# SonyResearch/COALA

Hardware: AMD Instinct MI355X
Metric: encode+decode GB/s over fp32 weight updates (device-resident), 1/2/4/8 GPU (higher is better)
Workload: dtype f32; 1 GPU; C3-per-GPU: 16 x resnet50_tv fp32 updates per GPU, top-k 0.01, 8-bit codes, weights mode, encode+decode batched as 2 concurrent sub-batches; layout=resnet50_tv, clients_per_gpu=16, elements_per_client=25610152, segments_per_client=267, mode=weights, global_clients=16, bits=8, inflight_steps=1, parallelism=replicas1

## Files before the change

coala_amd/compression/_lib.py:

```python
import ctypes
import os
import threading

from .. import _build

COALAC_FLAG_FORCE_EXACT = 1
COALAC_FLAG_GENERIC_SELECT = 2
COALAC_FLAG_STAMPS = 4
COALAC_FLAG_NO_FORK = 8
COALAC_AGG_DIV = 0
COALAC_AGG_RECIP = 1
COALAC_AGG_SUM = 2
COALAC_AGGD_CODES = 0
COALAC_AGGD_PACKED = 1
COALAC_AGGD_BLOCK = 2
COALAC_AGGS_ENTRIES = 0
COALAC_AGGS_COMPACT = 1
AGGD_DEPTH = 4

ERRORS = {
    -1: "COALAC_EINVAL",
    -2: "COALAC_EBITS",
    -3: "COALAC_EWORKSPACE",
    -4: "COALAC_EHIP",
    -5: "COALAC_EDEVICE",
    -6: "COALAC_ENOMEM",
}

_P = ctypes.c_void_p
_U64 = ctypes.c_uint64
_I = ctypes.c_int
SIGNATURES = [
    ("coalac_version", _I, []),
    ("coalac_last_error", ctypes.c_char_p, []),
    ("coalac_plan_create", _I, [_P, _I, _I, ctypes.POINTER(_P)]),
    ("coalac_plan_destroy", _I, [_P]),
    ("coalac_plan_query", _I, [_P, ctypes.POINTER(_U64), ctypes.POINTER(_U64), ctypes.POINTER(_U64),
                               ctypes.POINTER(_U64)]),
    ("coalac_encode", _I, [_P, _P, _P, _P, _P, _P, _P, _P, _P, _U64, ctypes.c_uint, _P]),
    ("coalac_encode_segptr", _I, [_P, _P, _P, _P, _P, _P, _P, _P, _P, _U64, ctypes.c_uint, _P]),
    ("coalac_decode", _I, [_P, _P, _P, _P, _P, _P, _P, _P, _P]),
    ("coalac_ef_accumulate", _I, [_P, _P, _P, _P, _P, _P]),
    ("coalac_ef_commit", _I, [_P, _P, _P, _P, _P, _P, _P, _P]),
    ("coalac_plan_packed_bytes", _I, [_P, ctypes.POINTER(_U64)]),
    ("coalac_pack", _I, [_P, _P, _P, _P, _U64, _P]),
    ("coalac_unpack", _I, [_P, _P, _U64, _P, _P, _P, _P]),
    ("coalac_plan_dense_packed_bytes", _I, [_P, ctypes.POINTER(_U64)]),
    ("coalac_pack_dense", _I, [_P, _P, _P, _U64, _P]),
    ("coalac_unpack_dense", _I, [_P, _P, _U64, _P, _P]),
    ("coalac_decode_packed", _I, [_P, _P, _U64, _P, _P, _P, _P, _P]),
    ("coalac_encode_block", _I, [_P, _P, _P, _P, _P, _P, _P, _U64, _P]),
    ("coalac_decode_block", _I, [_P, _P, _U64, _P, _P, _P, _P, _P]),
    ("coalac_encode_sr", _I, [_P, _P, _P, _P, _P, _P, _P, _P, _U64, _U64, ctypes.c_uint, _P]),
    ("coalac_encode_block_sr", _I, [_P, _P, _P, _P, _P, _P, _P, _U64, _U64, _P]),
    ("coalac_encode_ev", _I, [_P, _P, _P, _P, _P, _P, _P, _P, _P, _U64, ctypes.c_uint, _P, _P]),
    ("coalac_decode_ev", _I, [_P, _P, _P, _P, _P, _P, _P, _P, _P, _P]),
    ("coalac_aggregate", _I, [_P, _I, _P, _P, _P, _P, _P, _P, ctypes.c_float, _I, _P, _P, _P, _P]),
    ("coalac_aggregate_ev", _I, [_P, _I, _P, _P, _P, _P, _P, _P, ctypes.c_float, _I, _P, _P, _P, _P, _P]),
    ("coalac_aggregate_dense", _I, [_P, _I, _I, _P, _U64, _P, _P, _P, ctypes.c_float, _I, _P, _P, _P, _P]),
    ("coalac_aggregate_uploads", _I, [_P, _I, _I, _P, _P, _U64, _P, _P, _P, _P, _P, ctypes.c_float, _I, _P, _P, _P, _P]),
    ("coalac_gather", _I, [_P, _I, _I, _P, _P]),
    ("coalac_workspace_fallbacks", _I, [_P, _P, _P, ctypes.POINTER(_I)]),
    ("coalac_debug_stamps", _I, [_P, _P, _P, ctypes.POINTER(ctypes.c_uint64), _I]),
    ("coalac_debug_brackets", _I, [_P, _P, _P, ctypes.POINTER(ctypes.c_uint32), ctypes.POINTER(ctypes.c_uint32), _I]),
]

ABI_VERSION = 11
ADDED_IN_ABI_11 = ("coalac_encode_sr", "coalac_encode_block_sr")


class CodecError(RuntimeError):
    pass


class SegDesc(ctypes.Structure):
    _fields_ = [("in_off", _U64), ("n", _U64), ("k", _U64), ("out_off", _U64)]


_lock = threading.Lock()
_lib = None


def lib_path():
    return os.environ.get("COALAC_LIB") or _build.LIB


def load(build_if_missing=True):
    global _lib
    if _lib is not None:
        return _lib
    with _lock:
        if _lib is not None:
            return _lib
        path = lib_path()
        if not os.environ.get("COALAC_LIB") and (
                not os.path.exists(path) or (build_if_missing and _build.stale() and _can_build())):
            if not build_if_missing:
                raise CodecError(f"HIP codec library not found at {path}; run __graft_entry__.build()")
            _build.build()
        lib = ctypes.CDLL(path)
        lib.coalac_version.restype, lib.coalac_version.argtypes = _I, []
        v = lib.coalac_version()
        if v != ABI_VERSION:
            raise CodecError(f"libcoalac ABI version {v} != expected {ABI_VERSION} ({path}: rebuild it from this tree)")
        for name, res, args in SIGNATURES:
            if name in ADDED_IN_ABI_11 and not hasattr(lib, name):
                continue
            fn = getattr(lib, name)
            fn.restype = res
            fn.argtypes = args
        _lib = lib
        return lib


def _can_build():
    try:
        _build.hipcc()
        return True
    except RuntimeError:
        return False

# ... 6 lines not shown
```

coala_amd/compression/plan.py:

```python
import contextlib
import ctypes
from dataclasses import dataclass

import torch

from . import _lib
from .spec import RAW_BITS, UNIT, VALID_BITS, SegmentTable, SubTable


@dataclass
class Encoded:
    idx: torch.Tensor
    vals: torch.Tensor
    mn: torch.Tensor
    scale: torch.Tensor
    ustart: torch.Tensor = None
    packed: torch.Tensor = None

    FIELDS = ("idx", "vals", "mn", "scale", "ustart")

    def to(self, device, non_blocking=False):
        return Encoded(*(None if t is None else t.to(device, non_blocking=non_blocking)
                         for t in (self.idx, self.vals, self.mn, self.scale, self.ustart, self.packed)))

# ... 19 lines not shown

def _stream_handle(stream):
    s = torch.cuda.current_stream() if stream is None else stream
    return ctypes.c_void_p(s.cuda_stream)


class CodecPlan:

    def __init__(self, sizes, ratio, bits=8, clients=1, device=None, table=None):
        if bits not in VALID_BITS:
            raise ValueError(f"bits must be one of {VALID_BITS}, got {bits}")
        self.table = SegmentTable(sizes, ratio, clients) if table is None else table
        self.bits = int(bits)
        self.device = torch.device("cuda", torch.cuda.current_device() if device is None
                                   else torch.device(device).index or 0)
        self._lib = _lib.load()
        segs = self.table.segs
        arr = (_lib.SegDesc * len(segs))()
        for i, (a, b, c, d) in enumerate(segs.tolist()):
            arr[i] = _lib.SegDesc(a, b, c, d)
        h = ctypes.c_void_p()
        with torch.cuda.device(self.device):
            _lib.check(self._lib.coalac_plan_create(arr, len(segs), self.bits, ctypes.byref(h)),
                       "coalac_plan_create")
        self._h = h
        ws, tk, span, nu = (ctypes.c_uint64() for _ in range(4))
        _lib.check(self._lib.coalac_plan_query(h, ctypes.byref(ws), ctypes.byref(tk), ctypes.byref(span),
                                               ctypes.byref(nu)), "coalac_plan_query")
        self.ws_bytes = ws.value
        self.total_k, self.span, self.n_units = tk.value, span.value, nu.value
        if self.total_k != self.table.total_k:
            raise _lib.CodecError(f"plan total_k {self.total_k} != table {self.table.total_k}")
        if self.n_units != self.table.n_units:
            raise _lib.CodecError(f"plan n_units {self.n_units} != table {self.table.n_units}")
        segs = self.table.segs
        self.dense = bool(len(segs)) and bool((segs[:, 1] == segs[:, 2]).all())
        self.implied_idx = self.dense and getattr(self.table, "ratio", None) is not None and self.table.ratio >= 1.0

    @classmethod
    def from_segments(cls, segs, bits=8, device=None):
        return cls(None, None, bits, device=device, table=SubTable(segs))

    def close(self):
        h, self._h = getattr(self, "_h", None), None
        if h is not None and h.value:
            with torch.cuda.device(self.device):
                self._lib.coalac_plan_destroy(h)

    def __del__(self):
        try:
            self.close()
        except Exception:
            pass

    @property
    def n_segments(self):
        return self.table.n_segments

    @property
    def vals_dtype(self):
        return torch.float32 if self.bits == RAW_BITS else torch.uint8

    def empty_flat(self):
        return torch.empty(self.span, dtype=torch.float32, device=self.device)

    def empty_encoded(self, with_idx=None):
        if with_idx is None:
            with_idx = not self.implied_idx
        if not with_idx:
            vb = 4 if self.bits == RAW_BITS else 1
            T = self.n_segments
            buf = torch.empty((vb * self.total_k + 15) // 16 * 16 + 8 * T, dtype=torch.uint8, device=self.device)
            o = (vb * self.total_k + 15) // 16 * 16
            return Encoded(torch.empty(0, dtype=torch.int32, device=self.device), buf[:vb * self.total_k].view(self.vals_dtype),
                           buf[o:o + 4 * T].view(torch.float32), buf[o + 4 * T:o + 8 * T].view(torch.float32), None)
        geo = self.__dict__.get("_enc_geometry")
        if geo is None:
            K, T, U = self.total_k, self.n_segments, self.n_units
            vb = 4 if self.bits == RAW_BITS else 1
            views, o = [], 0
            dts = (torch.int32, self.vals_dtype, torch.float32, torch.float32, torch.int32)
            for nbytes, dt in zip((4 * K, vb * K, 4 * T, 4 * T, 4 * U), dts):
                views.append((o, nbytes, dt))
                o = (o + nbytes + 15) // 16 * 16
            geo = self._enc_geometry = (max(o, 16), tuple(views))
        buf = torch.empty(geo[0], dtype=torch.uint8, device=self.device)
        return Encoded(*[buf[a:a + n].view(dt) for a, n, dt in geo[1]])

    def empty_workspace(self):
        return torch.empty(self.ws_bytes, dtype=torch.uint8, device=self.device)

    def _check_flat(self, t, name, need=None):
        if t is None:
            return
        need = self.span if need is None else need
        if t.device != self.device or t.dtype != torch.float32 or not t.is_contiguous():
            raise ValueError(f"{name}: need a contiguous float32 tensor on {self.device}, got "
                             f"{t.dtype} on {t.device} (contiguous={t.is_contiguous()})")
        if t.numel() < need:
            raise ValueError(f"{name}: {t.numel()} elements < required {need}")
        if t.data_ptr() % 16:
            raise ValueError(f"{name}: storage must be 16-byte aligned")

    def _check_encoded(self, e):
        want = ((e.idx, torch.int32, 0 if self.dense and e.idx.numel() == 0 else self.total_k),
                (e.vals, self.vals_dtype, self.total_k),
# ... 567 lines not shown
```

coala_amd/csrc/coalac.hip:

```cpp
#pragma clang fp contract(off)

#include <hip/hip_runtime.h>

#include <algorithm>
#include <cmath>
#include <cstdarg>
#include <cstdio>
#include <cstdlib>
#include <cstring>
#include <mutex>
#include <string>
#include <type_traits>
#include <vector>

#include "../../include/coalac.h"

namespace {

constexpr int BLOCK = 256;
constexpr int WAVES = BLOCK / 64;
constexpr uint32_t UNIT = 4096;
constexpr uint32_t UNIT_SHIFT = 12;
constexpr uint32_t UNIT_IT = UNIT / 256;
constexpr uint32_t SMALL_MAX = 4096;
// ... 1806 lines not shown
    const uint32_t so = gx + qp;
    if (valid) {
      pst(P, P.eqpre + lb + i, ex);
      pst(P, P.outoff + lb + i, so);
      if (P.ustart_out != nullptr) pst(P, P.ustart_out + sd.unit_begin + i, so);
      const uint32_t rawu = raw_path | (zero_tie && quota > 0 ? 1u : 0u);
      P.uemit[lb + i] = make_uint4(T, rt | (rawu << 31), __float_as_uint(mn), __float_as_uint(scale));
    }
  }
}

template <int NT, bool DELTA, bool RAW>
DEV void segment_select(const Params& P, uint32_t li, SelSmem& S) {
  const uint32_t t = threadIdx.x;
  const uint32_t s = P.large_list[li];
  const SegDev sd = P.lsegs[li];
  const uint4 st = P.sstate[li];
  const uint32_t lb = sd.lu_begin, nu = sd.unit_end - sd.unit_begin;
  STAMP(P, li, 0);
  uint32_t T = 0, rt = 0, fp_rank = NONE, fn_rank = NONE;
  float gmn = qnan(), gmx = qnan();
  const bool zero_tie = st.w == 2;
  bool done;
  if (zero_tie) {
    const uint32_t g0 = sd.g_begin, ng = (nu + GU - 1) / GU;
    const uint32_t tk = P.tlo[lb] & KEY_MAX;
    gmn = t < ng ? P.gmm[2 * (g0 + t)] : qnan();
    gmx = t < ng ? P.gmm[2 * (g0 + t) + 1] : qnan();
    for (uint32_t i = t; i < nu; i += NT) S.ge[i] = P.gtC[lb + i] | (P.cntZ[lb + i] << 16);
    __syncthreads();
    T = tk;
    rt = st.z;
    fp_rank = rt > 0 ? 0u : NONE;
    if (tk != 0u) zero_tie_ranks<NT>(P, lb, nu, S, fp_rank, fn_rank);
    done = true;
  } else {
    done = st.w == 0 && select_from_groups<NT>(P, sd, lb, nu, st, S, T, rt, fp_rank, fn_rank, gmn, gmx);
  }
  uint32_t raw_path = 0;
  STAMP(P, li, 1);
  if (!done) select_fallback<NT, DELTA>(P, s, sd, S, T, rt, fp_rank, fn_rank, gmn, gmx, raw_path);
  STAMP(P, li, 10);
  select_finish<NT, RAW>(P, s, sd, S, done, zero_tie, raw_path, T, rt, fp_rank, fn_rank, gmn, gmx);
  STAMP(P, li, 12);
}

template <bool DELTA, bool RAW, int NT = SEL_NT>
__global__ __launch_bounds__(NT) void k_select(Params P) {
  __shared__ SelSmem S;
  segment_select<NT, DELTA, RAW>(P, blockIdx.x, S);
}

constexpr uint32_t EMIT_UPW = 4u;
constexpr uint32_t EMIT_UPW_LAT = 1u;

template <bool DELTA, bool RAW>
DEV void emit_raw_unit(const Params& P, const UnitDev& L, uint32_t T, uint32_t rt, uint32_t eqp, uint64_t obase,
                       float mn, float scale) {
  const uint32_t lane = lane_id();
  uint32_t eqc = 0, outc = 0;
  raw_unit_rows<DELTA>(P, L, [&](uint32_t row, float4 v) {
    const float xs[4] = {v.x, v.y, v.z, v.w};
    const uint32_t e0 = (row * 64 + lane) * 4;
    bool gt[4], tie[4], sel[4];
    uint32_t tpre = 0, spre = 0, ntie = 0, nsel = 0;
    uint64_t tb[4];
#pragma unroll
    for (int j = 0; j < 4; ++j) {
      const uint32_t key = fkey(xs[j]);
      const bool ok = e0 + j < L.len;
      gt[j] = ok && key > T;
      tie[j] = ok && key == T;
      tb[j] = __ballot(tie[j]);
      tpre += mbcnt(tb[j]);
      ntie += (uint32_t)__popcll(tb[j]);
    }
    uint32_t mine = 0;
#pragma unroll
    for (int j = 0; j < 4; ++j) {
      sel[j] = gt[j] || (tie[j] && eqp + eqc + tpre + mine < rt);
      mine += tie[j] ? 1u : 0u;
    }
    uint64_t sb[4];
#pragma unroll
    for (int j = 0; j < 4; ++j) {
      sb[j] = __ballot(sel[j]);
      spre += mbcnt(sb[j]);
      nsel += (uint32_t)__popcll(sb[j]);
    }
    uint32_t k = 0;
#pragma unroll
    for (int j = 0; j < 4; ++j) {
      if (sel[j]) {
        const uint64_t o = obase + outc + spre + k;
        P.idx[o] = (int32_t)(L.start + e0 + j);
        store_val<RAW>(P, o, xs[j], mn, scale);
        ++k;
      }
    }
    eqc += ntie;
    outc += nsel;
  });
}

template <bool DELTA, bool RAW, uint32_t UPW, uint32_t TR>
DEV void emit_units(const Params& P, uint32_t lu0, uint32_t lu1, uint32_t stride) {
  const uint32_t lane = lane_id();
  auto unit = [&](uint32_t g) { return lu0 + g * stride; };
  const uint32_t ng = lu0 < lu1 ? min(UPW, (lu1 - lu0 + stride - 1) / stride) : 0u;
  const uint32_t lug = unit(min(lane, ng - 1));
  uint32_t nCg, startg, eqpg, oog, Tg, rtg, stg;
  uint64_t sog;
  float mng, scg;
  uint2 rec0[UPW];
  if constexpr (UPW == 1) {
    const uint32_t nCr = P.cntC[lug];
    startg = P.lunits[lug].start;
    sog = P.lunits[lug].out_off;
    eqpg = P.eqpre[lug];
    oog = P.outoff[lug];
    const uint4 ue = P.uemit[lug];
    const uint64_t r0 = (uint64_t)lu0 * P.ccap;
    rec0[0] = make_uint2(P.cpos[r0 + lane], P.cval[r0 + lane]);
    nCg = min(nCr, P.ccap);
    Tg = ue.x;
    rtg = ue.y & 0x7FFFFFFFu;
    stg = ue.y >> 31;
    mng = RAW ? 0.0f : __uint_as_float(ue.z);
    scg = RAW ? 0.0f : __uint_as_float(ue.w);
  } else {
    nCg = min(P.cntC[lug], P.ccap);
    startg = P.lunits[lug].start;
    sog = P.lunits[lug].out_off;
    eqpg = P.eqpre[lug];
    oog = P.outoff[lug];
    const uint4 ue = P.uemit[lug];
    Tg = ue.x;
    rtg = ue.y & 0x7FFFFFFFu;
    stg = ue.y >> 31;
    mng = RAW ? 0.0f : __uint_as_float(ue.z);
    scg = RAW ? 0.0f : __uint_as_float(ue.w);
#pragma unroll
    for (uint32_t g = 0; g < UPW; ++g) {
      const uint32_t lu = unit(min(g, ng - 1)), nC = rl(nCg, g);
      const uint32_t last = nC ? nC - 1 : 0u;
      const uint64_t r0 = (uint64_t)lu * P.ccap;
      rec0[g] = make_uint2(P.cpos[r0 + min(lane, last)], P.cval[r0 + min(lane, last)]);
    }
  }
#pragma unroll
  for (uint32_t g = 0; g < UPW; ++g) {
    const uint32_t nC = rl(nCg, g);
    if (g < ng && rl(stg, g) != 0) {
      const uint64_t so = ((uint64_t)rl((uint32_t)(sog >> 32), g) << 32) | rl((uint32_t)sog, g);
      emit_raw_unit<DELTA, RAW>(P, P.lunits[unit(g)], rl(Tg, g), rl(rtg, g), rl(eqpg, g), so + rl(oog, g),
                                __uint_as_float(rl(__float_as_uint(mng), g)), __uint_as_float(rl(__float_as_uint(scg), g)));
    } else if (g < ng && nC != 0) {
      const uint32_t lu = unit(g);
      const uint32_t T = rl(Tg, g), rt = rl(rtg, g), eqp = rl(eqpg, g);
      const float mn = __uint_as_float(rl(__float_as_uint(mng), g));
      const float scale = __uint_as_float(rl(__float_as_uint(scg), g));
      const uint64_t so = ((uint64_t)rl((uint32_t)(sog >> 32), g) << 32) | rl((uint32_t)sog, g);
      const uint64_t obase = so + rl(oog, g);
      const uint32_t start = rl(startg, g);
      const uint64_t r0 = (uint64_t)lu * P.ccap;
      uint32_t eqc = 0, outc = 0;
      auto row = [&](uint32_t i0, uint2 rec) {
        const uint32_t i = i0 + lane;
        const bool valid = i < nC;
        const float x = __uint_as_float(rec.y);
        const uint32_t key = fkey(x);
        const bool e = valid && key == T;
        const uint64_t eb = __ballot(e);
        const uint32_t rank = eqp + eqc + mbcnt(eb);
        eqc += (uint32_t)__popcll(eb);
        const bool sel = valid && (key > T || (e && rank < rt));
        const uint64_t sb = __ballot(sel);
        if (sel) {
          const uint64_t o = obase + outc + mbcnt(sb);
          P.idx[o] = (int32_t)(start + rec.x);
          store_val<RAW>(P, o, x, mn, scale);
        }
        outc += (uint32_t)__popcll(sb);
      };
      row(0, rec0[g]);
      for (uint32_t i0 = 64; i0 < nC; i0 += 64 * TR) {
        uint2 rb[TR];
#pragma unroll
        for (uint32_t b = 0; b < TR; ++b) {
          const uint32_t ic = min(i0 + b * 64 + lane, nC - 1);
          if (i0 + b * 64 < nC) rb[b] = make_uint2(P.cpos[r0 + ic], P.cval[r0 + ic]);
        }
#pragma unroll
        for (uint32_t b = 0; b < TR; ++b)
          if (i0 + b * 64 < nC) row(i0 + b * 64, rb[b]);
      }
    }
  }
}

template <bool DELTA, bool RAW, uint32_t UPW, uint32_t TR>
__global__ __launch_bounds__(BLOCK) void k_emit(Params P) {
  const uint32_t wv = threadIdx.x >> 6;
  const uint32_t t0 = blockIdx.x * WAVES * UPW;
  if (t0 + wv >= P.n_lunits) return;
  const bool st = blockIdx.x < P.nseg;
  if (st) STAMP(P, blockIdx.x, 13);
  emit_units<DELTA, RAW, UPW, TR>(P, t0 + wv, min(t0 + WAVES * UPW, P.n_lunits), WAVES);
  if (st) STAMP(P, blockIdx.x, 14);
}

constexpr int DECODE_LDS_WPE = 5;
constexpr int DECODE_LDS_WPE_BASE = 4;
constexpr uint32_t DECODE_QROWS = 8u;
constexpr uint32_t DECODE_QROWS_BASE = 4u;
constexpr int DECODE_NT = 256;
constexpr uint32_t DECODE_WPU_LAT = 2u;
constexpr int DECODE_SAUX_LAT = 0;

template <bool RAW, bool HASBASE, uint32_t WPU, uint32_t QROWS, int SAUX, bool XCD, uint32_t NCH = 1>
__global__ __launch_bounds__(DECODE_NT, HASBASE ? DECODE_LDS_WPE_BASE : DECODE_LDS_WPE) void k_decode_lds(Params P) {
  constexpr uint32_t DW = DECODE_NT / 64, RPW = UNIT_IT / WPU, NPASS = RPW / QROWS;
  constexpr uint32_t QSH = QROWS == 2u ? 9u : QROWS == 4u ? 10u : QROWS == 8u ? 11u : 12u, QM = (1u << QSH) - 1u;
  static_assert((QROWS << 8) == (1u << QSH) && RPW % QROWS == 0 && NPASS >= 1, "tile pass geometry");
  __shared__ float4 qtile[DW][QROWS * 64];
  const uint32_t lane = lane_id(), wv = threadIdx.x >> 6;
  const uint32_t wid = (XCD ? xcd_block(blockIdx.x) : blockIdx.x) * DW + wv;
  const uint32_t u = wid / WPU, pass0 = (wid % WPU) * NPASS;
  if (u >= P.n_units) return;
  float4* tile = qtile[wv];
  float* tf = reinterpret_cast<float*>(tile);
#pragma unroll
  for (uint32_t it = 0; it < QROWS; ++it) tile[it * 64 + lane] = make_float4(0.0f, 0.0f, 0.0f, 0.0f);
  const UnitDev U = P.units[u];
  uint32_t lo = P.ustart[u];
  uint32_t hi = P.ustart[min(u + 1, P.n_units - 1)];
  const float mn = RAW ? 0.0f : P.cmn[U.seg], sc = RAW ? 0.0f : P.cscale[U.seg];
  lo = min(lo, U.k);
  hi = max(lo, min(min(U.last ? U.k : hi, U.k), lo + U.len));
// ... 1336 lines not shown
  std::vector<uint4> groups, gseg;
};

size_t place_tables(const PlanTables& T, Params& P, uint8_t* host, const uint8_t* dev) {
  Carver c{host};
  auto put = [&](auto*& dst, const auto& v) {
    using E = typename std::decay_t<decltype(v)>::value_type;
    static_assert(std::is_same<decltype(dst), const E*&>::value, "table and pointer types differ");
    E* h = c.take<E>(v.size());
    if (!host) return;
    if (!v.empty()) memcpy(h, v.data(), sizeof(E) * v.size());
    dst = reinterpret_cast<const E*>(dev + (reinterpret_cast<uint8_t*>(h) - host));
  };
  put(P.segs, T.segs);
  put(P.units, T.units);
  put(P.lunits, T.lunits);
  put(P.small_list, T.small_list);
  put(P.large_list, T.large_list);
  put(P.lsegs, T.lsegs);
  put(P.ssegs, T.ssegs);
  put(P.groups, T.groups);
  put(P.gseg, T.gseg);
  return c.off + 256;
}

template <typename F>
auto with_flags(F&& f) {
  return f();
}
template <typename F, typename... Rest>
auto with_flags(F&& f, bool flag, Rest... rest) {
  if (flag) return with_flags([&](auto... t) { return f(std::true_type{}, t...); }, rest...);
  return with_flags([&](auto... t) { return f(std::false_type{}, t...); }, rest...);
}
template <typename F>
auto with_agg_mode(int mode, F&& f) {
  if (mode == COALAC_AGG_RECIP) return f(std::integral_constant<int, COALAC_AGG_RECIP>{});
  if (mode == COALAC_AGG_SUM) return f(std::integral_constant<int, COALAC_AGG_SUM>{});
  return f(std::integral_constant<int, COALAC_AGG_DIV>{});
}

constexpr uint32_t FORK_MIN_LUNITS = 16384;

}

struct coalac_plan {
  int device = -1;
  int bits = 8;
  bool dense = false;
  bool dense_empty = false;
  bool encode_latency = false;
  bool decode_latency = false;
  bool high_ratio = false;
  bool small_1k = false;
  bool fork_sized = false;
  uint64_t span = 0, total_k = 0, ws_bytes = 0;
  uint64_t dense_words = 0;
  const uint64_t* dense_pw = nullptr;
  Params proto{};
  void* meta = nullptr;
  std::vector<SegDev> hsegs;
  hipStream_t side = nullptr;
  hipEvent_t fork = nullptr, join = nullptr;
  std::mutex mu;
};

namespace {

int check_device(coalac_plan_t plan) {
  int dev = -1;
  HIP_CHECK(hipGetDevice(&dev));
  if (dev != plan->device)
    return fail(COALAC_EDEVICE, "current device %d differs from the plan's device %d", dev, plan->device);
  return COALAC_OK;
}

uintptr_t addr_bits(const void* a, const void* b = nullptr, const void* c = nullptr) {
  return reinterpret_cast<uintptr_t>(a) | reinterpret_cast<uintptr_t>(b) | reinterpret_cast<uintptr_t>(c);
}

void set_payload(Params& P, const int32_t* d_idx, const void* d_vals, const float* d_mn, const float* d_scale) {
  P.cidx = d_idx;
  P.cvals = d_vals;
  P.cmn = d_mn;
  P.cscale = d_scale;
}

int launched() {
  HIP_CHECK(hipGetLastError());
  return COALAC_OK;
}

struct Marks {
  void* const* ev;
  int n;
  int at(int i, hipStream_t st) const {
    if (ev != nullptr && i < n && ev[i] != nullptr) HIP_CHECK(hipEventRecord(static_cast<hipEvent_t>(ev[i]), st));
    return COALAC_OK;
  }
};

#define MARK(i)                         \
  do {                                  \
    const int rc_ = marks.at((i), st);  \
    if (rc_) return rc_;                \
  } while (0)
// ... 44 lines not shown
    lk.lock();
    if (plan->side == nullptr) {
      if (hipStreamCreateWithFlags(&plan->side, hipStreamNonBlocking) != hipSuccess ||
          hipEventCreateWithFlags(&plan->fork, hipEventDisableTiming) != hipSuccess ||
          hipEventCreateWithFlags(&plan->join, hipEventDisableTiming) != hipSuccess)
        return fail(COALAC_EHIP, "creating the plan's side stream / events failed: %s",
                    hipGetErrorString(hipGetLastError()));
    }
  }
  MARK(0);
  if (fork) {
    HIP_CHECK(hipEventRecord(plan->fork, st));
    HIP_CHECK(hipStreamWaitEvent(plan->side, plan->fork, 0));
    hipLaunchKernelGGL((k_small<DELTA, RAW>), dim3(P.n_small), dim3(BLOCK), 0, plan->side, P);
    HIP_CHECK(hipEventRecord(plan->join, plan->side));
  }
  if (presel && !small_in_scan)
    hipLaunchKernelGGL((k_presel<DELTA, RAW>), dim3(P.n_large + P.n_small), dim3(BLOCK), 0, st, P);
  else if (P.n_large && lat)
    hipLaunchKernelGGL((k_sample<DELTA, RAW, SAMPLE_NT_LAT>), dim3(P.n_large), dim3(SAMPLE_NT_LAT), 0, st, P);
  else if (P.n_large)
    hipLaunchKernelGGL((k_sample<DELTA, RAW, BLOCK>), dim3(P.n_large), dim3(BLOCK), 0, st, P);
  MARK(1);
  if (small_in_scan) {
    Q.scan_small = P.n_small;
    const dim3 gs(ceil_div(P.n_lunits, SCAN_NT_LAT / 64) + P.n_small);
    if (plan->small_1k)
      hipLaunchKernelGGL((k_scan<DELTA, RAW, true, SCAN_WPE_LAT_1K, SCAN_NB_LAT, SCAN_NT_LAT, SMALL_MAX_LATENCY>), gs,
                         dim3(SCAN_NT_LAT), 0, st, Q);
    else
      hipLaunchKernelGGL((k_scan<DELTA, RAW, true, SCAN_WPE_LAT, SCAN_NB_LAT, SCAN_NT_LAT>), gs, dim3(SCAN_NT_LAT), 0, st,
                         Q);
  } else if (P.n_lunits) {
    hipLaunchKernelGGL((k_scan<DELTA, RAW, false, SCAN_WPE, SCAN_NB, SCAN_NT>), dim3(ceil_div(P.n_lunits, SCAN_NT / 64)),
                       dim3(SCAN_NT), 0, st, Q);
  }
  MARK(2);
  if (P.n_large && lat) {
    hipLaunchKernelGGL((k_ghist<GHIST_NT_LAT, true>), dim3(P.n_groups), dim3(GHIST_NT_LAT), 0, st, P);
    hipLaunchKernelGGL((k_gwin<GWIN_NT_LAT, true>), dim3(P.n_groups), dim3(GWIN_NT_LAT), 0, st, P);
    hipLaunchKernelGGL((k_select<DELTA, RAW, SEL_NT_LAT>), dim3(P.n_large), dim3(SEL_NT_LAT), 0, st, P);
  } else if (P.n_large) {
    with_flags(
        [&](auto hr) {
          hipLaunchKernelGGL((k_ghist<BLOCK, false, hr.value>), dim3(P.n_groups), dim3(BLOCK), 0, st, P);
          hipLaunchKernelGGL((k_gwin<BLOCK, false, hr.value>), dim3(P.n_groups), dim3(BLOCK), 0, st, P);
        },
        plan->high_ratio);
    hipLaunchKernelGGL((k_select<DELTA, RAW>), dim3(P.n_large), dim3(SEL_NT), 0, st, P);
  }
  MARK(3);
  if (P.n_large)
    with_flags(
        [&](auto l, auto hr) {
          constexpr uint32_t UPW = l.value ? EMIT_UPW_LAT : EMIT_UPW, TR = hr.value ? 4u : 1u;
          hipLaunchKernelGGL((k_emit<DELTA, RAW, UPW, TR>), dim3(ceil_div(P.n_lunits, UPW * WAVES)), dim3(BLOCK), 0, st, P);
        },
        lat, plan->high_ratio);
  if (fork) HIP_CHECK(hipStreamWaitEvent(st, plan->join, 0));
  MARK(4);
  return COALAC_OK;
}

int encode_impl(coalac_plan_t plan, const float* d_in, const float* const* d_inptr, const float* d_base,
                int32_t* d_idx, void* d_vals, float* d_mn, float* d_scale, uint32_t* d_ustart, void* d_ws,
                uint64_t ws_bytes, unsigned flags, void* stream, const Marks& marks) {
  if (!plan) return fail(COALAC_EINVAL, "coalac_encode: plan is NULL");
  if (plan->proto.nseg == 0) return COALAC_OK;
  if (!d_mn || !d_scale) return fail(COALAC_EINVAL, "coalac_encode: mn/scale pointers are NULL");
  if (plan->span && !d_in && !d_inptr) return fail(COALAC_EINVAL, "coalac_encode: input pointer is NULL");
  if (plan->total_k && (!(d_idx || plan->dense) || !d_vals))
    return fail(COALAC_EINVAL, "coalac_encode: idx/vals pointers are NULL (idx may be NULL for a dense plan only)");
  if (addr_bits(d_in, d_base) & 15) return fail(COALAC_EINVAL, "coalac_encode: input/base must be 16-byte aligned");
  if (addr_bits(d_ustart) & 3) return fail(COALAC_EINVAL, "coalac_encode: ustart must be 4-byte aligned");
  if (!d_ws || ws_bytes < plan->ws_bytes)
    return fail(COALAC_EWORKSPACE, "coalac_encode: workspace %llu < required %llu", (unsigned long long)ws_bytes,
                (unsigned long long)plan->ws_bytes);
  int rc = check_device(plan);
  if (rc) return rc;
  Params P = plan->proto;
  P.in = d_in;
  P.inptr = d_inptr;
  P.base = d_base;
  P.idx = d_idx;
  P.vals = d_vals;
  P.mn = d_mn;
  P.scale = d_scale;
  P.ustart_out = d_ustart;
  P.flags = flags;
  carve_workspace(P, plan->dense, d_ws);
  if (!(flags & COALAC_FLAG_STAMPS)) P.stamps = nullptr;
  hipStream_t st = static_cast<hipStream_t>(stream);
  rc = with_flags(
      [&](auto delta, auto raw) {
        return plan->dense ? launch_dense_encode<delta.value, raw.value>(P, plan, st, marks)
                           : launch_encode<delta.value, raw.value>(P, plan, st, marks);
      },
      d_base != nullptr, plan->bits == 32);
  return rc ? rc : launched();
}

template <bool RAW, bool HB, bool HR>
void launch_decode_lds(const Params& P, coalac_plan_t plan, hipStream_t st) {
  constexpr uint32_t DW = DECODE_NT / 64, NCH = HR ? 8u : 1u;
  if (plan->decode_latency) {
    constexpr uint32_t W = DECODE_WPU_LAT, Q = HB ? DECODE_QROWS_BASE : UNIT_IT / DECODE_WPU_LAT;
    hipLaunchKernelGGL((k_decode_lds<RAW, HB, W, (Q < 8u ? Q : 8u), DECODE_SAUX_LAT, false, NCH>),
                       dim3(ceil_div(P.n_units * W, DW)), dim3(DECODE_NT), 0, st, P);
  } else {
    hipLaunchKernelGGL((k_decode_lds<RAW, HB, 1u, HB ? DECODE_QROWS_BASE : DECODE_QROWS, STORE_AUX, true, NCH>),
                       dim3(ceil_div(P.n_units, DW)), dim3(DECODE_NT), 0, st, P);
// ... 116 lines not shown
      for (uint32_t g0 = 0; g0 < nu; g0 += GU) {
        T.groups.push_back(make_uint4((uint32_t)T.large_list.size(), d.lu_begin + g0, std::min(GU, nu - g0), (uint32_t)s));
        T.gseg.push_back(make_uint4(d.lu_begin, nu, (uint32_t)g.k, d.g_begin));
      }
    }
    (large ? T.large_list : T.small_list).push_back((uint32_t)s);
    (large ? T.lsegs : T.ssegs).push_back(d);
    T.segs[s] = d;
    if (g.n) {
      span = std::max<uint64_t>(span, g.in_off + g.n);
      total_k = std::max<uint64_t>(total_k, g.out_off + g.k);
      in_r.push_back({g.in_off, g.in_off + g.n});
      out_r.push_back({g.out_off, g.out_off + g.k});
    }
  }
  if (T.lunits.size() >= (1ull << 32) / UNIT)
    return fail(COALAC_EINVAL, "plan too large (%zu large units)", T.lunits.size());
  auto overlaps = [](std::vector<std::pair<uint64_t, uint64_t>>& r) {
    std::sort(r.begin(), r.end());
    for (size_t i = 1; i < r.size(); ++i)
      if (r[i].first < r[i - 1].second) return true;
    return false;
  };
  if (overlaps(in_r)) return fail(COALAC_EINVAL, "segment input ranges overlap");
  if (overlaps(out_r)) return fail(COALAC_EINVAL, "segment output ranges overlap");

  int dev = 0;
  HIP_CHECK(hipGetDevice(&dev));
  coalac_plan* p = new coalac_plan();
  p->device = dev;
  p->bits = bits;
  p->span = span;
  p->total_k = total_k;
  p->hsegs = T.segs;
  Params& M = p->proto;
  M.nseg = (uint32_t)nseg;
  M.n_small = (uint32_t)T.small_list.size();
  M.n_large = (uint32_t)T.large_list.size();
  M.n_units = (uint32_t)T.units.size();
  M.n_lunits = (uint32_t)T.lunits.size();
  M.n_groups = (uint32_t)T.groups.size();
  M.levels = bits == 32 ? 0.0f : (float)((1u << bits) - 1u);
  double rmax = 0.0;
  for (const SegDev& d : T.lsegs) rmax = std::max(rmax, (double)d.k / (double)d.n);
  uint32_t ccap = (uint32_t)align_up((size_t)(UNIT * std::min(1.0, 2.0 * rmax + 0.05) + 256.0), 64);
  if (const char* e = getenv("COALAC_CCAP")) ccap = (uint32_t)atoi(e);
  M.ccap = std::max<uint32_t>(STAGE_CAP, std::min<uint32_t>(UNIT, ccap));
  p->dense = true;
  for (const SegDev& d : T.segs) p->dense = p->dense && d.k == d.n;
  for (const SegDev& d : T.segs) p->dense_empty = p->dense_empty || d.unit_begin == d.unit_end;
  p->encode_latency = M.n_lunits <= LATENCY_PLAN_UNITS;
  p->decode_latency = decode_latency;
  p->high_ratio = rmax > HIGH_RATIO;
  p->small_1k = small_max <= SMALL_MAX_LATENCY;
  p->fork_sized = M.n_small && M.n_lunits >= FORK_MIN_LUNITS;
  p->ws_bytes = carve_workspace(M, p->dense, nullptr);
  std::vector<uint64_t> dense_pw;
  if (p->dense && bits != 32) {
    dense_pw.reserve(T.segs.size());
    for (const SegDev& d : T.segs) {
      dense_pw.push_back(p->dense_words);
      p->dense_words += ((uint64_t)d.n * (uint64_t)bits + 31u) / 32u;
    }
  }

  const size_t tables = place_tables(T, M, nullptr, nullptr);
  const size_t bytes = tables + align_up(sizeof(uint64_t) * dense_pw.size(), 256);
  std::vector<uint8_t> host(bytes, 0);
  hipError_t e = hipMalloc(&p->meta, bytes);
  if (e != hipSuccess) {
    delete p;
    return fail(COALAC_ENOMEM, "hipMalloc(%zu) for plan metadata failed: %s", bytes, hipGetErrorString(e));
  }
  place_tables(T, M, host.data(), static_cast<const uint8_t*>(p->meta));
  if (!dense_pw.empty()) {
    memcpy(host.data() + tables, dense_pw.data(), sizeof(uint64_t) * dense_pw.size());
    p->dense_pw = reinterpret_cast<const uint64_t*>(static_cast<const uint8_t*>(p->meta) + tables);
  }
  e = hipMemcpy(p->meta, host.data(), bytes, hipMemcpyHostToDevice);
  if (e != hipSuccess) {
    (void)hipFree(p->meta);
    delete p;
    return fail(COALAC_EHIP, "hipMemcpy of plan metadata failed: %s", hipGetErrorString(e));
  }
  *out = p;
  return COALAC_OK;
}

int coalac_plan_destroy(coalac_plan_t plan) {
  if (!plan) return COALAC_OK;
  int cur = 0;
  if (hipGetDevice(&cur) == hipSuccess && cur != plan->device) (void)hipSetDevice(plan->device);
  hipError_t e = hipFree(plan->meta);
  if (plan->side) (void)hipStreamDestroy(plan->side);
  if (plan->fork) (void)hipEventDestroy(plan->fork);
  if (plan->join) (void)hipEventDestroy(plan->join);
  if (cur != plan->device) (void)hipSetDevice(cur);
  delete plan;
  if (e != hipSuccess) return fail(COALAC_EHIP, "hipFree failed: %s", hipGetErrorString(e));
  return COALAC_OK;
}

int coalac_plan_query(coalac_plan_t plan, uint64_t* ws_bytes, uint64_t* total_k, uint64_t* span, uint64_t* n_units) {
  if (!plan) return fail(COALAC_EINVAL, "coalac_plan_query: plan is NULL");
  if (ws_bytes) *ws_bytes = plan->ws_bytes;
  if (total_k) *total_k = plan->total_k;
  if (span) *span = plan->span;
  if (n_units) *n_units = plan->proto.n_units;
  return COALAC_OK;
}

int coalac_encode_ev(coalac_plan_t plan, const float* d_in, const float* d_base, int32_t* d_idx,
                     void* d_vals, float* d_mn, float* d_scale, uint32_t* d_ustart, void* d_ws, uint64_t ws_bytes,
                     unsigned flags, void* stream, void* const* events) {
  return encode_impl(plan, d_in, nullptr, d_base, d_idx, d_vals, d_mn, d_scale, d_ustart, d_ws, ws_bytes, flags, stream,
                     Marks{events, 5});
}

int coalac_encode_segptr(coalac_plan_t plan, const float* const* d_seg_in, const float* d_base, int32_t* d_idx,
                         void* d_vals, float* d_mn, float* d_scale, uint32_t* d_ustart, void* d_ws, uint64_t ws_bytes,
                         unsigned flags, void* stream) {
  if (plan && plan->proto.nseg && !d_seg_in) return fail(COALAC_EINVAL, "coalac_encode_segptr: d_seg_in is NULL");
  return encode_impl(plan, nullptr, d_seg_in, d_base, d_idx, d_vals, d_mn, d_scale, d_ustart, d_ws, ws_bytes, flags,
                     stream, Marks{nullptr, 0});
}

int coalac_encode(coalac_plan_t plan, const float* d_in, const float* d_base, int32_t* d_idx, void* d_vals,
                  float* d_mn, float* d_scale, uint32_t* d_ustart, void* d_ws, uint64_t ws_bytes, unsigned flags,
                  void* stream) {
  return coalac_encode_ev(plan, d_in, d_base, d_idx, d_vals, d_mn, d_scale, d_ustart, d_ws, ws_bytes, flags, stream,
                          nullptr);
}

int coalac_decode_ev(coalac_plan_t plan, const int32_t* d_idx, const void* d_vals, const float* d_mn,
                     const float* d_scale, const uint32_t* d_ustart, const float* d_base, float* d_out, void* stream,
                     void* const* events) {
  if (!plan) return fail(COALAC_EINVAL, "coalac_decode: plan is NULL");
  if (plan->proto.n_units == 0) return COALAC_OK;
  if (!d_out) return fail(COALAC_EINVAL, "coalac_decode: output pointer is NULL");
  if (plan->total_k && (!(plan->dense || (d_idx && d_ustart)) || !d_vals))
    return fail(COALAC_EINVAL, "coalac_decode: idx/vals/ustart pointers are NULL (a sparse plan needs the per-unit "
                "starts of wire v2)");
  if (plan->total_k && plan->bits != 32 && (!d_mn || !d_scale))
    return fail(COALAC_EINVAL, "coalac_decode: mn/scale pointers are NULL");
  if (addr_bits(d_out, d_base) & 15) return fail(COALAC_EINVAL, "coalac_decode: output/base must be 16-byte aligned");
  if (addr_bits(d_ustart) & 3) return fail(COALAC_EINVAL, "coalac_decode: ustart must be 4-byte aligned");
  int rc = check_device(plan);
  if (rc) return rc;
  Params P = plan->proto;
  set_payload(P, d_idx, d_vals, d_mn, d_scale);
  P.base = d_base;
  P.out = d_out;
  P.ustart = d_ustart;
  hipStream_t st = static_cast<hipStream_t>(stream);
  const bool raw = plan->bits == 32, hb = d_base != nullptr;
  const Marks marks{events, 3};
  MARK(0);
  MARK(1);
  if (plan->dense)
    with_flags(
        [&](auto r, auto h, auto x) {
// ... 522 lines not shown
```

include/coalac.h:

```cpp
#ifndef COALAC_H
#define COALAC_H

#include <stdint.h>

#ifdef __cplusplus
extern "C" {
#endif

#define COALAC_ABI_VERSION 11

enum {
  COALAC_OK = 0,
  COALAC_EINVAL = -1,
  COALAC_EBITS = -2,
  COALAC_EWORKSPACE = -3,
  COALAC_EHIP = -4,
  COALAC_EDEVICE = -5,
  COALAC_ENOMEM = -6
};

enum {
  COALAC_FLAG_FORCE_EXACT = 1,
  COALAC_FLAG_GENERIC_SELECT = 2,
  COALAC_FLAG_STAMPS = 4,
  COALAC_FLAG_NO_FORK = 8
};

typedef struct coalac_seg {
  uint64_t in_off;
  uint64_t n;
  uint64_t k;
  uint64_t out_off;
} coalac_seg_t;

typedef struct coalac_plan* coalac_plan_t;

int coalac_version(void);
const char* coalac_last_error(void);

int coalac_plan_create(const coalac_seg_t* h_segs, int nseg, int bits, coalac_plan_t* out);
int coalac_plan_destroy(coalac_plan_t plan);

int coalac_plan_query(coalac_plan_t plan, uint64_t* ws_bytes, uint64_t* total_k, uint64_t* span, uint64_t* n_units);

int coalac_encode(coalac_plan_t plan, const float* d_in, const float* d_base, int32_t* d_idx,
                  void* d_vals, float* d_mn, float* d_scale, uint32_t* d_ustart, void* d_ws, uint64_t ws_bytes,
                  unsigned flags, void* stream);

int coalac_encode_segptr(coalac_plan_t plan, const float* const* d_seg_in, const float* d_base, int32_t* d_idx,
                         void* d_vals, float* d_mn, float* d_scale, uint32_t* d_ustart, void* d_ws, uint64_t ws_bytes,
                         unsigned flags, void* stream);

int coalac_decode(coalac_plan_t plan, const int32_t* d_idx, const void* d_vals, const float* d_mn,
                  const float* d_scale, const uint32_t* d_ustart, const float* d_base, float* d_out, void* stream);

int coalac_ef_accumulate(coalac_plan_t plan, const float* d_in, const float* const* d_seg_in, const float* d_base,
                         float* d_resid, void* stream);
int coalac_ef_commit(coalac_plan_t plan, const int32_t* d_idx, const void* d_vals, const float* d_mn,
                     const float* d_scale, const uint32_t* d_ustart, float* d_resid, void* stream);

int coalac_plan_packed_bytes(coalac_plan_t plan, uint64_t* bytes);
int coalac_pack(coalac_plan_t plan, const int32_t* d_idx, const void* d_vals, void* d_packed, uint64_t packed_bytes,
                void* stream);
int coalac_unpack(coalac_plan_t plan, const void* d_packed, uint64_t packed_bytes, const uint32_t* d_ustart,
                  int32_t* d_idx, void* d_vals, void* stream);

int coalac_plan_dense_packed_bytes(coalac_plan_t plan, uint64_t* bytes);
int coalac_pack_dense(coalac_plan_t plan, const void* d_vals, void* d_packed, uint64_t packed_bytes, void* stream);
int coalac_unpack_dense(coalac_plan_t plan, const void* d_packed, uint64_t packed_bytes, void* d_vals, void* stream);
int coalac_decode_packed(coalac_plan_t plan, const void* d_packed, uint64_t packed_bytes, const float* d_mn,
                         const float* d_scale, const float* d_base, float* d_out, void* stream);

int coalac_encode_block(coalac_plan_t plan, const float* d_in, const float* const* d_seg_in, const float* d_base,
                        float* d_bmn, float* d_bscale, void* d_packed, uint64_t packed_bytes, void* stream);
int coalac_decode_block(coalac_plan_t plan, const void* d_packed, uint64_t packed_bytes, const float* d_bmn,
                        const float* d_bscale, const float* d_base, float* d_out, void* stream);

int coalac_encode_sr(coalac_plan_t plan, const float* d_in, const float* const* d_seg_in, const float* d_base,
                     void* d_vals, float* d_mn, float* d_scale, void* d_ws, uint64_t ws_bytes, uint64_t seed,
                     unsigned flags, void* stream);
int coalac_encode_block_sr(coalac_plan_t plan, const float* d_in, const float* const* d_seg_in, const float* d_base,
                           float* d_bmn, float* d_bscale, void* d_packed, uint64_t packed_bytes, uint64_t seed,
                           void* stream);

int coalac_encode_ev(coalac_plan_t plan, const float* d_in, const float* d_base, int32_t* d_idx,
                     void* d_vals, float* d_mn, float* d_scale, uint32_t* d_ustart, void* d_ws, uint64_t ws_bytes,
                     unsigned flags, void* stream, void* const* events);
int coalac_decode_ev(coalac_plan_t plan, const int32_t* d_idx, const void* d_vals, const float* d_mn,
                     const float* d_scale, const uint32_t* d_ustart, const float* d_base, float* d_out, void* stream,
                     void* const* events);

enum { COALAC_AGG_DIV = 0, COALAC_AGG_RECIP = 1, COALAC_AGG_SUM = 2 };
int coalac_aggregate(coalac_plan_t plan, int clients, const int32_t* d_idx, const void* d_vals,
                     const float* d_mn, const float* d_scale, const uint32_t* d_ustart, const float* d_weights,
                     float total, int mode, const uint8_t* d_avg_mask, const float* d_base, float* d_out,
                     void* stream);
// ... 32 lines not shown
```

Before: 2790 GB/s.

## Make emit units-per-wave selectable and prefetch candidate rows speculatively

The emit kernel's units-per-wave becomes a per-plan setting (default 2, overridable via env var or API) instead of the fixed 4, which raises the number of blocks launched. For multi-unit waves, the first two 64-wide candidate rows of every unit are now loaded up front without bounds clamping, and the high-ratio extra rows are prefetched before the emit loop. This is meant to hide global-load latency behind earlier issue. It costs more registers per thread, which may reduce occupancy.

```diff
diff --git a/coala_amd/compression/_lib.py b/coala_amd/compression/_lib.py
--- a/coala_amd/compression/_lib.py
+++ b/coala_amd/compression/_lib.py
@@ -37,6 +37,8 @@
     ("coalac_plan_destroy", _I, [_P]),
     ("coalac_plan_query", _I, [_P, ctypes.POINTER(_U64), ctypes.POINTER(_U64), ctypes.POINTER(_U64),
                                ctypes.POINTER(_U64)]),
+    ("coalac_plan_emit_upw", _I, [_P, ctypes.POINTER(_I), ctypes.POINTER(_I)]),
+    ("coalac_plan_set_emit_upw", _I, [_P, _I]),
     ("coalac_encode", _I, [_P, _P, _P, _P, _P, _P, _P, _P, _P, _U64, ctypes.c_uint, _P]),
     ("coalac_encode_segptr", _I, [_P, _P, _P, _P, _P, _P, _P, _P, _P, _U64, ctypes.c_uint, _P]),
     ("coalac_decode", _I, [_P, _P, _P, _P, _P, _P, _P, _P, _P]),
@@ -66,7 +68,7 @@
 ]
 
 ABI_VERSION = 11
-ADDED_IN_ABI_11 = ("coalac_encode_sr", "coalac_encode_block_sr")
+ADDED_IN_ABI_11 = ("coalac_encode_sr", "coalac_encode_block_sr", "coalac_plan_emit_upw", "coalac_plan_set_emit_upw")
 
 
 class CodecError(RuntimeError):
diff --git a/coala_amd/compression/plan.py b/coala_amd/compression/plan.py
--- a/coala_amd/compression/plan.py
+++ b/coala_amd/compression/plan.py
@@ -95,6 +95,30 @@
             self.close()
         except Exception:
             pass
+
+    EMIT_UPW_CHOICES = (2, 4, 8)
+
+    def _emit_query(self):
+        fn = getattr(self._lib, "coalac_plan_emit_upw", None)
+        if fn is None:
+            raise _lib.CodecError("the loaded codec library has no coalac_plan_emit_upw (built before the plan field)")
+        upw, batch = ctypes.c_int(), ctypes.c_int()
+        _lib.check(fn(self._h, ctypes.byref(upw), ctypes.byref(batch)), "coalac_plan_emit_upw")
+        return upw.value, bool(batch.value)
+
+    @property
+    def emit_upw(self):
+        return self._emit_query()[0]
+
+    @emit_upw.setter
+    def emit_upw(self, upw):
+        if int(upw) not in self.EMIT_UPW_CHOICES:
+            raise ValueError(f"emit_upw must be one of {self.EMIT_UPW_CHOICES}, got {upw}")
+        _lib.check(self._lib.coalac_plan_set_emit_upw(self._h, int(upw)), "coalac_plan_set_emit_upw")
+
+    @property
+    def encode_batch(self):
+        return self._emit_query()[1]
 
     @property
     def n_segments(self):
diff --git a/coala_amd/csrc/coalac.hip b/coala_amd/csrc/coalac.hip
--- a/coala_amd/csrc/coalac.hip
+++ b/coala_amd/csrc/coalac.hip
@@ -1882,6 +1882,13 @@
 }
 
 constexpr uint32_t EMIT_UPW = 4u;
+inline uint32_t emit_upw_for(bool high_ratio, double kept_per_unit, uint32_t ccap) {
+  (void)high_ratio;
+  (void)kept_per_unit;
+  (void)ccap;
+  return 2u;
+}
+constexpr uint32_t EMIT_SPEC_ROWS = 2u;
 constexpr uint32_t EMIT_UPW_LAT = 1u;
 
 template <bool DELTA, bool RAW>
@@ -1942,7 +1949,9 @@
   uint32_t nCg, startg, eqpg, oog, Tg, rtg, stg;
   uint64_t sog;
   float mng, scg;
-  uint2 rec0[UPW];
+  constexpr uint32_t SR = UPW == 1 ? 1u : EMIT_SPEC_ROWS;
+  uint2 rec0[UPW][SR];
+  uint2 rec1[UPW][TR];
   if constexpr (UPW == 1) {
     const uint32_t nCr = P.cntC[lug];
     startg = P.lunits[lug].start;
@@ -1951,7 +1960,7 @@
     oog = P.outoff[lug];
     const uint4 ue = P.uemit[lug];
     const uint64_t r0 = (uint64_t)lu0 * P.ccap;
-    rec0[0] = make_uint2(P.cpos[r0 + lane], P.cval[r0 + lane]);
+    rec0[0][0] = make_uint2(P.cpos[r0 + lane], P.cval[r0 + lane]);
     nCg = min(nCr, P.ccap);
     Tg = ue.x;
     rtg = ue.y & 0x7FFFFFFFu;
@@ -1959,23 +1968,38 @@
     mng = RAW ? 0.0f : __uint_as_float(ue.z);
     scg = RAW ? 0.0f : __uint_as_float(ue.w);
   } else {
-    nCg = min(P.cntC[lug], P.ccap);
+    uint32_t nCr = P.cntC[lug];
     startg = P.lunits[lug].start;
     sog = P.lunits[lug].out_off;
     eqpg = P.eqpre[lug];
     oog = P.outoff[lug];
     const uint4 ue = P.uemit[lug];
+#pragma unroll
+    for (uint32_t g = 0; g < UPW; ++g) {
+      const uint64_t r0 = (uint64_t)unit(min(g, ng - 1)) * P.ccap;
+#pragma unroll
+      for (uint32_t b = 0; b < SR; ++b)
+        rec0[g][b] = make_uint2(P.cpos[r0 + b * 64 + lane], P.cval[r0 + b * 64 + lane]);
+    }
+    uint32_t uy = ue.y;
+    asm volatile("" : "+v"(nCr), "+v"(uy)::"memory");
+    nCg = min(nCr, P.ccap);
     Tg = ue.x;
-    rtg = ue.y & 0x7FFFFFFFu;
-    stg = ue.y >> 31;
+    rtg = uy & 0x7FFFFFFFu;
+    stg = uy >> 31;
     mng = RAW ? 0.0f : __uint_as_float(ue.z);
     scg = RAW ? 0.0f : __uint_as_float(ue.w);
 #pragma unroll
     for (uint32_t g = 0; g < UPW; ++g) {
-      const uint32_t lu = unit(min(g, ng - 1)), nC = rl(nCg, g);
-      const uint32_t last = nC ? nC - 1 : 0u;
-      const uint64_t r0 = (uint64_t)lu * P.ccap;
-      rec0[g] = make_uint2(P.cpos[r0 + min(lane, last)], P.cval[r0 + min(lane, last)]);
+      const uint32_t nC = rl(nCg, g);
+      if (g < ng && rl(stg, g) == 0 && nC > 64 * SR) {
+        const uint64_t r0 = (uint64_t)unit(g) * P.ccap;
+#pragma unroll
+        for (uint32_t b = 0; b < TR; ++b) {
+          const uint32_t ic = min(64 * (SR + b) + lane, nC - 1);
+          rec1[g][b] = make_uint2(P.cpos[r0 + ic], P.cval[r0 + ic]);
+        }
+      }
     }
   }
 #pragma unroll
@@ -2013,8 +2037,17 @@
         }
         outc += (uint32_t)__popcll(sb);
       };
-      row(0, rec0[g]);
-      for (uint32_t i0 = 64; i0 < nC; i0 += 64 * TR) {
+#pragma unroll
+      for (uint32_t b = 0; b < SR; ++b)
+        if (b * 64 < nC) row(b * 64, rec0[g][b]);
+      if constexpr (UPW != 1) {
+        if (nC > 64 * SR) {
+#pragma unroll
+          for (uint32_t b = 0; b < TR; ++b)
+            if (64 * (SR + b) < nC) row(64 * (SR + b), rec1[g][b]);
+        }
+      }
+      for (uint32_t i0 = 64 * (UPW == 1 ? 1u : SR + TR); i0 < nC; i0 += 64 * TR) {
         uint2 rb[TR];
 #pragma unroll
         for (uint32_t b = 0; b < TR; ++b) {
@@ -3457,6 +3490,7 @@
   bool encode_latency = false;
   bool decode_latency = false;
   bool high_ratio = false;
+  uint32_t emit_upw = EMIT_UPW;
   bool small_1k = false;
   bool fork_sized = false;
   uint64_t span = 0, total_k = 0, ws_bytes = 0;
@@ -3607,11 +3641,12 @@
   MARK(3);
   if (P.n_large)
     with_flags(
-        [&](auto l, auto hr) {
-          constexpr uint32_t UPW = l.value ? EMIT_UPW_LAT : EMIT_UPW, TR = hr.value ? 4u : 1u;
+        [&](auto l, auto hr, auto wide, auto widest) {
+          constexpr uint32_t UPW = l.value ? EMIT_UPW_LAT : !wide.value ? 2u : widest.value ? 8u : 4u;
+          constexpr uint32_t TR = hr.value ? 4u : 1u;
           hipLaunchKernelGGL((k_emit<DELTA, RAW, UPW, TR>), dim3(ceil_div(P.n_lunits, UPW * WAVES)), dim3(BLOCK), 0, st, P);
         },
-        lat, plan->high_ratio);
+        lat, plan->high_ratio, plan->emit_upw >= 4u, plan->emit_upw == 8u);
   if (fork) HIP_CHECK(hipStreamWaitEvent(st, plan->join, 0));
   MARK(4);
   return COALAC_OK;
@@ -3834,6 +3869,13 @@
   p->encode_latency = M.n_lunits <= LATENCY_PLAN_UNITS;
   p->decode_latency = decode_latency;
   p->high_ratio = rmax > HIGH_RATIO;
+  uint64_t kept_large = 0;
+  for (const SegDev& d : T.lsegs) kept_large += d.k;
+  p->emit_upw = emit_upw_for(p->high_ratio, M.n_lunits ? (double)kept_large / (double)M.n_lunits : 0.0, M.ccap);
+  if (const char* e = getenv("COALAC_EMIT_UPW")) {
+    const int v = atoi(e);
+    if (v == 2 || v == 4 || v == 8) p->emit_upw = (uint32_t)v;
+  }
   p->small_1k = small_max <= SMALL_MAX_LATENCY;
   p->fork_sized = M.n_small && M.n_lunits >= FORK_MIN_LUNITS;
   p->ws_bytes = carve_workspace(M, p->dense, nullptr);
@@ -3889,6 +3931,21 @@
   if (total_k) *total_k = plan->total_k;
   if (span) *span = plan->span;
   if (n_units) *n_units = plan->proto.n_units;
+  return COALAC_OK;
+}
+
+int coalac_plan_emit_upw(coalac_plan_t plan, int* upw, int* batch) {
+  if (!plan) return fail(COALAC_EINVAL, "coalac_plan_emit_upw: plan is NULL");
+  if (upw) *upw = (int)plan->emit_upw;
+  if (batch) *batch = plan->encode_latency ? 0 : 1;
+  return COALAC_OK;
+}
+
+int coalac_plan_set_emit_upw(coalac_plan_t plan, int upw) {
+  if (!plan) return fail(COALAC_EINVAL, "coalac_plan_set_emit_upw: plan is NULL");
+  if (upw != 2 && upw != 4 && upw != 8) return fail(COALAC_EINVAL, "coalac_plan_set_emit_upw: upw=%d (2, 4 or 8)", upw);
+  std::lock_guard<std::mutex> lk(plan->mu);
+  plan->emit_upw = (uint32_t)upw;
   return COALAC_OK;
 }
 
diff --git a/include/coalac.h b/include/coalac.h
--- a/include/coalac.h
+++ b/include/coalac.h
@@ -42,6 +42,9 @@
 int coalac_plan_destroy(coalac_plan_t plan);
 
 int coalac_plan_query(coalac_plan_t plan, uint64_t* ws_bytes, uint64_t* total_k, uint64_t* span, uint64_t* n_units);
+
+int coalac_plan_emit_upw(coalac_plan_t plan, int* upw, int* batch);
+int coalac_plan_set_emit_upw(coalac_plan_t plan, int upw);
 
 int coalac_encode(coalac_plan_t plan, const float* d_in, const float* d_base, int32_t* d_idx,
                   void* d_vals, float* d_mn, float* d_scale, uint32_t* d_ustart, void* d_ws, uint64_t ws_bytes,
```

Result: no change. 2791 GB/s (median of 2 runs) (+0.0%).
